# althonos/lightmotif

Hardware: AMD Instinct MI355X
Metric: scored positions/sec (higher is better)
Workload: dtype f32

## Files before the change

lightmotif_amd/build.py:

```python
from __future__ import annotations

import os
import shutil
import subprocess
import sys
from concurrent.futures import ThreadPoolExecutor
from pathlib import Path

PKG = Path(__file__).resolve().parent
CSRC = PKG / "csrc"
ROOT = PKG.parent
OBJ = CSRC / "_obj"
LIB = CSRC / "liblightmotif_hip.so"

ARCH = "gfx950"
FLAGS = [f"--offload-arch={ARCH}", "-O3", "-std=c++17", "-fPIC", "-ffp-contract=off",
         "-fno-slp-vectorize", "-fno-fast-math", "-Wall", "-Wno-unused-function",
         f"-I{ROOT / 'include'}", f"-I{CSRC}"]
INST = [(i, 4 * i + 1, 4 * i + 4) for i in range(9)]
LONG = list(range(40, 65, 4))
LONG_FLAGS = ["-mllvm", "-pragma-unroll-threshold=10000000"]
XLONG = list(range(72, 89, 8))
PAIR = [(65, 80), (81, 96), (97, 112), (113, 128)]
UNITS = ["score_plan.hip", "score_store.hip", "score_argmax.hip", "score_threshold.hip", "reduce.hip", "hits.hip", "seqset.hip", "seqset_best.hip", "fasta.hip", "dist.hip", "discrete.hip", "layout.hip", "scanmax.hip", "context.hip", "pssm.hip", "score_api.hip", "handles.hip",
         "hostptr.hip", "comm.hip"]
UNIT_FLAGS = {"seqset_best.hip": LONG_FLAGS}


def _hipcc() -> str:
    exe = shutil.which("hipcc") or "/opt/rocm/bin/hipcc"
    if not os.path.exists(exe):
        raise RuntimeError("hipcc not found: the HIP back-end cannot be built")
    return exe


def _newer(target: Path, deps: list[Path]) -> bool:
    if not target.exists():
        return True
    t = target.stat().st_mtime
    return any(d.stat().st_mtime > t for d in deps)


def _run(cmd: list[str]) -> None:
    r = subprocess.run(cmd, stdout=subprocess.PIPE, stderr=subprocess.STDOUT, text=True)
    if r.returncode != 0:
        raise RuntimeError("command failed: " + " ".join(cmd) + "\n" + r.stdout)
    if r.stdout.strip() and os.environ.get("LM_BUILD_VERBOSE"):
        print(r.stdout)


def build(force: bool = False, jobs: int | None = None) -> Path:
    hipcc = _hipcc()
    OBJ.mkdir(exist_ok=True)
    headers = list(CSRC.glob("*.hpp")) + [ROOT / "include" / "lightmotif_hip.h", Path(__file__)]
    cmds, objs = [], []
    for unit in UNITS:
        obj = OBJ / (unit + ".o")
        objs.append(obj)
        if force or _newer(obj, [CSRC / unit] + headers):
            cmds.append([hipcc, *FLAGS, *UNIT_FLAGS.get(unit, []), "-c", str(CSRC / unit), "-o", str(obj)])
    for inst, lo, hi in INST:
        obj = OBJ / f"score_inst_{inst}.o"
        objs.append(obj)
        if force or _newer(obj, [CSRC / "score_inst.hip"] + headers):
            cmds.append([hipcc, *FLAGS, f"-DLM_M_LO={lo}", f"-DLM_M_HI={hi}", f"-DLM_INST_ID={inst}",
                         "-c", str(CSRC / "score_inst.hip"), "-o", str(obj)])
    for m in LONG:
        obj = OBJ / f"score_long_inst_{m}.o"
        objs.append(obj)
        if force or _newer(obj, [CSRC / "score_long_inst.hip"] + headers):
            cmds.append([hipcc, *FLAGS, *LONG_FLAGS, f"-DLM_LONG_M={m}", "-c", str(CSRC / "score_long_inst.hip"),
                         "-o", str(obj)])
    for m in XLONG:
        obj = OBJ / f"score_xlong_inst_{m}.o"
        objs.append(obj)
        if force or _newer(obj, [CSRC / "score_xlong_inst.hip"] + headers):
            cmds.append([hipcc, *FLAGS, *LONG_FLAGS, f"-DLM_XLONG_M={m}", "-c", str(CSRC / "score_xlong_inst.hip"),
                         "-o", str(obj)])
    for lo, hi in PAIR:
        obj = OBJ / f"score_pair_inst_{lo}.o"
        objs.append(obj)
        if force or _newer(obj, [CSRC / "score_pair_inst.hip"] + headers):
            cmds.append([hipcc, *FLAGS, *LONG_FLAGS, f"-DLM_PAIR_LO={lo}", f"-DLM_PAIR_HI={hi}", "-c",
                         str(CSRC / "score_pair_inst.hip"), "-o", str(obj)])
    if cmds:
        def weight(cmd):
            text = " ".join(cmd)
            for m in LONG:
                if f"-DLM_LONG_M={m}" in text:
                    return 1000 + m
            for m in XLONG:
                if f"-DLM_XLONG_M={m}" in text:
                    return 900 + m
            for inst, lo, hi in INST:
                if f"-DLM_INST_ID={inst}" in text:
                    return 100 + hi
            if "score_pair_inst.hip" in text:
                return 90
            return 50 if "score_" in text else 0
        cmds.sort(key=weight, reverse=True)
        with ThreadPoolExecutor(max_workers=jobs or min(8, os.cpu_count() or 1)) as ex:
            list(ex.map(_run, cmds))
    if cmds or force or not LIB.exists():
        _run([hipcc, f"--offload-arch={ARCH}", "-shared", "-fPIC", "-o", str(LIB),
              *map(str, objs), "-ldl"])
        _audit(LIB)
    return LIB


# ... 15 lines not shown
```

lightmotif_amd/csrc/context.hip:

```cpp
#include <algorithm>
#include <sys/mman.h>
#include <cmath>
#include <cstdarg>
#include <cstdio>
#include <cstdlib>
#include <cctype>
#include <cstring>
#include <new>
#include <string>

#include "score_registry.hpp"

#include "lm_internal.hpp"

namespace lm {

static thread_local char g_err[512] = "";

int fail(int status, const char *fmt, ...)
{
    va_list ap;
    va_start(ap, fmt);
    vsnprintf(g_err, sizeof g_err, fmt, ap);
    va_end(ap);
// ... 213 lines not shown
    if (pinned_in_use) *pinned_in_use = used;
    if (budget) *budget = pool_budget();
    return LM_HIP_OK;
}

size_t lm_hip_stride(size_t cols, size_t elem_size)
{
    if (elem_size == 0)
        return 0;
    const size_t bytes = (cols * elem_size + 31) / 32 * 32;
    return bytes / elem_size;
}


namespace lm {
__global__ void clock_probe_kernel(unsigned long long window_ticks, unsigned long long *out)
{
    const unsigned long long r0 = __builtin_amdgcn_s_memrealtime();
    const unsigned long long c0 = __builtin_amdgcn_s_memtime();
    unsigned long long r1 = r0;
    while (r1 - r0 < window_ticks) {
        __builtin_amdgcn_s_sleep(127);
        r1 = __builtin_amdgcn_s_memrealtime();
    }
    const unsigned long long c1 = __builtin_amdgcn_s_memtime();
    if (threadIdx.x == 0) {
        out[0] = c1 - c0;
        out[1] = r1 - r0;
    }
}
}

int lm_hip_device_clock_mhz(int device, unsigned window_us, double *mhz)
{
    if (!mhz)
        return fail(LM_HIP_ERR_BAD_ARGS, "device_clock_mhz: null output");
    *mhz = 0.0;
    if (window_us == 0 || window_us > 2000000u)
        return fail(LM_HIP_ERR_BAD_ARGS, "device_clock_mhz: window of %u us (1 ... 2 000 000)", window_us);
    int n = 0;
    if (hipGetDeviceCount(&n) != hipSuccess || device < 0 || device >= n)
        return fail(LM_HIP_ERR_NO_DEVICE, "device %d out of range (%d devices)", device, n);
    DeviceGuard guard(device);
    int wall_khz = 0;
    LM_HIP_TRY(hipDeviceGetAttribute(&wall_khz, hipDeviceAttributeWallClockRate, device));
    if (wall_khz <= 0)
        return fail(LM_HIP_ERR_HIP, "device_clock_mhz: the device reports no constant-rate counter");
    struct Probe {
        hipStream_t stream = nullptr;
        unsigned long long *rec = nullptr;
    };
    static std::mutex probe_mu;
    static Probe probes[64];
    std::lock_guard<std::mutex> probe_lock(probe_mu);
    if (device >= 64)
        return fail(LM_HIP_ERR_BAD_ARGS, "device_clock_mhz: device ordinal %d", device);
    Probe &pr = probes[device];
    hipError_t e = hipSuccess;
    if (!pr.stream)
        e = hipStreamCreateWithFlags(&pr.stream, hipStreamNonBlocking);
    if (e == hipSuccess && !pr.rec)
        e = hipHostMalloc(reinterpret_cast<void **>(&pr.rec), 2 * sizeof(unsigned long long), hipHostMallocDefault);
    if (e == hipSuccess) {
        pr.rec[0] = pr.rec[1] = 0;
        hipLaunchKernelGGL(clock_probe_kernel, dim3(1), dim3(64), 0, pr.stream,
                           (unsigned long long)window_us * (unsigned long long)wall_khz / 1000ull, pr.rec);
        e = hipGetLastError();
    }
    if (e == hipSuccess)
        e = hipStreamSynchronize(pr.stream);
    const unsigned long long ticks = pr.rec ? pr.rec[0] : 0, ref = pr.rec ? pr.rec[1] : 0;
    if (e != hipSuccess)
        return fail(LM_HIP_ERR_HIP, "device_clock_mhz: %s", hipGetErrorString(e));
    if (ref == 0)
        return fail(LM_HIP_ERR_HIP, "device_clock_mhz: the constant-rate counter did not advance");
    *mhz = (double)ticks / (double)ref * (double)wall_khz / 1000.0;
    return LM_HIP_OK;
}


static const char *const kOptionNames[] = {"track_argmax", "xlong_store", "host_fold", "speculate_order", "suffix_argmax",
                                           "multi_motif", "quad_loads", "skip_unreachable", "pair_prefilter",
                                           "pair_prefilter_protein", "chunked_fused", "chunk_rows", "tiled",
                                           "suffix_occurrences", "prefilter", "sort_hits", "short_order", "time_scan", "drop_last", "block_prefilter", "list_scan_max", "poll_done"};

static int set_option(lm_hip_ctx *ctx, const char *name, double value)
{
    const bool on = value != 0;
    const std::string n(name);
    if (n == "track_argmax") ctx->track_argmax = on;
    else if (n == "xlong_store") ctx->xlong_store = on;
    else if (n == "host_fold") ctx->host_fold = on;
    else if (n == "speculate_order") ctx->speculate_order = on;
    else if (n == "sort_hits") ctx->sort_hits = on;
    else if (n == "time_scan") ctx->time_scan = on;
    else if (n == "poll_done") ctx->poll_done = on;
    else if (n == "list_scan_max") ctx->list_scan_max = on;
    else if (n == "drop_last") ctx->drop_last = on;
    else if (n == "short_order") ctx->short_order = on;
    else if (n == "suffix_argmax") ctx->suffix_argmax = on;
    else if (n == "multi_motif") ctx->multi_motif = on;
    else if (n == "quad_loads") ctx->quad_loads = on;
    else if (n == "skip_unreachable") ctx->skip_unreachable = on;
    else if (n == "pair_prefilter") ctx->pair_prefilter = on;
    else if (n == "block_prefilter") ctx->block_prefilter = on;
    else if (n == "pair_prefilter_protein") ctx->pair_prefilter_protein = on;
    else if (n == "chunked_fused") ctx->chunked_fused = on;
    else if (n == "tiled") ctx->tiled = on;
    else if (n == "prefilter") ctx->use_prefilter = on;
    else if (n == "xcd_remap") (void)on;
    else if (n == "chunk_rows") {
        if (!(value >= 64) || !(value <= 2147483648.0))
            return fail(LM_HIP_ERR_BAD_ARGS, "ctx_set_option: chunk_rows must be 64 ... 2^31");
        ctx->chunk_rows = (size_t)value;
    } else if (n == "suffix_occurrences") {
        ctx->suffix_occurrences = value > 0 ? value : 0;
    } else {
        return fail(LM_HIP_ERR_BAD_ARGS, "ctx_set_option: unknown option '%s'", name);
    }
    return LM_HIP_OK;
}

static void read_dev_switches(lm_hip_ctx *ctx)
{
#ifdef LM_HIP_DEV_SWITCHES
    for (const char *name : kOptionNames) {
        std::string env = "LM_HIP_";
        for (const char *c = name; *c; ++c)
            env += (char)toupper(*c);
        if (const char *e = getenv(env.c_str()))
            (void)set_option(ctx, name, atof(e));
    }
#else
    (void)ctx;
    (void)kOptionNames;
#endif
}

static int ctx_create(int device, void *stream, bool borrow, lm_hip_ctx **out)
{
    if (!out)
        return fail(LM_HIP_ERR_BAD_ARGS, "ctx_create: null output");
    *out = nullptr;
    if (const char *hole = score_registry_hole())
        return fail(LM_HIP_ERR_HIP, "%s", hole);
    int n = 0;
    if (hipGetDeviceCount(&n) != hipSuccess || n == 0)
        return fail(LM_HIP_ERR_NO_DEVICE, "no HIP device available");
    if (device < 0 || device >= n)
        return fail(LM_HIP_ERR_NO_DEVICE, "device %d out of range (%d devices)", device, n);
    hipDeviceProp_t prop;
    LM_HIP_TRY(hipGetDeviceProperties(&prop, device));
    if (strncmp(prop.gcnArchName, "gfx950", 6) != 0)
        return fail(LM_HIP_ERR_NO_DEVICE, "device %d is %s; this library is built for gfx950 only",
                    device, prop.gcnArchName);
    DeviceGuard guard(device);
    if (!guard.ok)
        return fail(LM_HIP_ERR_HIP, "hipSetDevice(%d) failed", device);
    lm_hip_ctx *ctx = new (std::nothrow) lm_hip_ctx();
    if (!ctx)
        return fail(LM_HIP_ERR_OOM, "out of host memory");
    ctx->device = device;
    ctx->num_cus = prop.multiProcessorCount;
    read_dev_switches(ctx);
    if (borrow) {
        ctx->stream = static_cast<hipStream_t>(stream);
        ctx->owns_stream = false;
    } else {
        hipError_t e = hipStreamCreateWithFlags(&ctx->stream, hipStreamNonBlocking);
        if (e != hipSuccess) {
            delete ctx;
            return fail(LM_HIP_ERR_HIP, "hipStreamCreate failed: %s", hipGetErrorString(e));
        }
        ctx->owns_stream = true;
    }
    hipError_t e = hipHostMalloc(&ctx->pinned, kPinnedBytes, hipHostMallocDefault);
    if (e != hipSuccess) {
        if (ctx->owns_stream)
            (void)hipStreamDestroy(ctx->stream);
        delete ctx;
        return fail(LM_HIP_ERR_OOM, "hipHostMalloc failed: %s", hipGetErrorString(e));
    }
    *out = ctx;
    return LM_HIP_OK;
// ... 151 lines not shown
```

lightmotif_amd/csrc/lm_internal.hpp:

```cpp
#pragma once

#include <hip/hip_runtime.h>

#include <cstddef>
#include <cstdint>
#include <mutex>
#include <string>
#include <vector>

#include "lightmotif_hip.h"

namespace lm {


int fail(int status, const char *fmt, ...) __attribute__((format(printf, 2, 3)));

#define LM_HIP_TRY(expr)                                                               \
    do {                                                                               \
        hipError_t _e = (expr);                                                        \
        if (_e != hipSuccess)                                                          \
            return ::lm::fail(_e == hipErrorOutOfMemory ? LM_HIP_ERR_OOM : LM_HIP_ERR_HIP, \
                              "%s failed: %s (%s:%d)", #expr, hipGetErrorString(_e),   \
                              __FILE__, __LINE__);                                     \
    } while (0)
// ... 19 lines not shown
    {
        if (prev >= 0)
            (void)hipSetDevice(prev);
    }
};


struct Scratch {
    void *ptr = nullptr;
    size_t bytes = 0;
    int reserve(size_t n);
    void release();
    void forget() { ptr = nullptr; bytes = 0; }
};

struct ArgmaxRecord {
    float value;
    int found;
    long long index;
};

constexpr size_t kPinnedBytes = 4u << 20;
struct PinnedRegion {
    size_t off, cap;
    constexpr size_t end() const { return off + cap; }
};
constexpr PinnedRegion kPinCounters{0, 16};
constexpr PinnedRegion kPinRecord{0, 64};
constexpr size_t kPinGenerationWordOff = sizeof(ArgmaxRecord);
constexpr PinnedRegion kPinArgmaxBatch{0, kPinnedBytes};
constexpr PinnedRegion kPinCandResults{16, kPinnedBytes / 2 - 16};
constexpr PinnedRegion kPinScanMaxState{0, 256};
constexpr PinnedRegion kPinListHead{256, kPinnedBytes / 2 - 256};
constexpr PinnedRegion kPinHitStaging{0, kPinnedBytes / 2};
constexpr PinnedRegion kPinHitReadback{0, 256u << 10};
constexpr PinnedRegion kPinFoldRecords{4096, kPinnedBytes - 4096};
constexpr PinnedRegion kPinU8Out{4096, kPinnedBytes / 2 - 4096};
constexpr PinnedRegion kPinUploadHead{kPinnedBytes / 2, kPinnedBytes / 2};
constexpr PinnedRegion kPinCommBlock{0, kPinnedBytes};
constexpr PinnedRegion kPinCommGather{0, kPinnedBytes / 2};

static_assert(kPinRecord.end() <= kPinFoldRecords.off, "single-job argmax: the record and its generation word lie before the wavefront records");
static_assert(kPinCounters.end() <= kPinCandResults.off, "candidate-route argmax: the counters lie before the results");
static_assert(kPinCandResults.end() <= kPinUploadHead.off, "candidate-route argmax: the results end where the uploaded head begins");
static_assert(kPinCounters.end() <= kPinListHead.off, "Scanner::max by list: the counters lie before the head of the list");
static_assert(kPinHitStaging.end() <= kPinUploadHead.off, "fused threshold: the kernels' staging ends where the uploaded head begins");
static_assert(kPinHitReadback.end() <= kPinHitStaging.end(), "the exact ordering's read-back stays inside the staging of the speculative one");
static_assert(kPinListHead.end() <= kPinUploadHead.off && kPinU8Out.end() <= kPinUploadHead.off, "the lower half's users stay in the lower half");

void *result_alloc(size_t bytes);
void result_free(void *p);

}


struct lm_hip_ctx {
    int device = 0;
    hipStream_t stream = nullptr;
    bool owns_stream = false;
    hipStream_t aux_stream = nullptr;
    hipEvent_t fork_event = nullptr, join_event = nullptr;
    hipStream_t copy_stream = nullptr;
    hipEvent_t tile_copied[2] = {nullptr, nullptr}, tile_consumed[2] = {nullptr, nullptr};
    std::mutex mu;
    lm::Scratch scratch;
    lm::Scratch scratch2;
    lm::Scratch scan_buf;
    lm::Scratch chunk_scores;
    size_t chunk_rows = 1u << 22;
    bool chunked_fused = true;
    void *pinned = nullptr;
    unsigned fold_generation = 0;
    unsigned *d_ticket = nullptr;
    unsigned *d_short = nullptr;
    unsigned short_generation = 0;
    bool poll_done = false;
    bool short_dirty = false;
    size_t rows_per_stream = 0;
    bool use_prefilter = true;
    bool pair_prefilter = true;
    bool block_prefilter = true;
    bool pair_prefilter_protein = false;
    bool quad_loads = true;
    bool track_argmax = true;
    bool xlong_store = true;
    bool host_fold = true;
    bool speculate_order = true;
    bool sort_hits = true;
    bool time_scan = false;
    hipEvent_t scan_ev[4] = {nullptr, nullptr, nullptr, nullptr};
    bool scan_timed = false;
    int scan_marks = 0;
    float last_scan_kernel_ms = -1.0f;
    float last_phase_ms[4] = {-1.0f, -1.0f, -1.0f, -1.0f};
    unsigned last_scan_rows = 0, last_scan_lds_bytes = 0;
    bool list_scan_max = true;
    bool drop_last = true;
    bool short_order = true;
    bool suffix_argmax = true;
    bool multi_motif = true;
    bool skip_unreachable = true;
    bool tiled = true;
    double suffix_occurrences = 0;
    int num_cus = 256;
    unsigned long long last_hit_count = 0;
    unsigned long long last_cand_count = 0;
    const char *last_kernel = "";
    lm::Scratch u8_tables;
    std::vector<uint8_t> u8_key;
};

namespace lm {
template <class T>
inline T *pinned_at(const lm_hip_ctx *ctx, PinnedRegion r, size_t count = 1, size_t byte_off = 0)
{
    if (byte_off + count * sizeof(T) > r.cap)
        return nullptr;
    return reinterpret_cast<T *>(static_cast<char *>(ctx->pinned) + r.off + byte_off);
}

template <class T>
inline int read_back(lm_hip_ctx *ctx, hipStream_t st, const void *d_src, T *out)
{
    static_assert(sizeof(T) <= kPinCounters.cap, "read_back is for a counter");
    T *h = pinned_at<T>(ctx, kPinCounters);
    LM_HIP_TRY(hipMemcpyAsync(h, d_src, sizeof(T), hipMemcpyDeviceToHost, st));
    LM_HIP_TRY(hipStreamSynchronize(st));
    *out = *h;
    return LM_HIP_OK;
}
inline int read_back_counters(lm_hip_ctx *ctx, hipStream_t st, const void *d_counters, unsigned long long out[2])
{
    struct Pair { unsigned long long hits, candidates; } p{};
    LM_TRY(read_back(ctx, st, d_counters, &p));
    out[0] = p.hits;
    out[1] = p.candidates;
    return LM_HIP_OK;
}

inline unsigned next_generation(unsigned &g) { return ++g ? g : ++g; }
inline bool poll_generation(const volatile unsigned *word, unsigned generation, unsigned spins = 1u << 20)
{
    for (unsigned spin = 0; spin < spins; ++spin) {
        if (__atomic_load_n(word, __ATOMIC_ACQUIRE) == generation)
            return true;
#if defined(__x86_64__) && !defined(__HIP_DEVICE_COMPILE__)
        __builtin_ia32_pause();
#endif
    }
    return false;
}
struct FoldSlots {
    uint4 *records;
    unsigned generation;
};
inline FoldSlots begin_fold(lm_hip_ctx *ctx, size_t nrec, bool want_records = true)
{
    FoldSlots f{want_records ? pinned_at<uint4>(ctx, kPinFoldRecords, nrec + 1) : nullptr, next_generation(ctx->fold_generation)};
    if (f.records)
        for (size_t r = 0; r <= nrec; ++r)
            reinterpret_cast<volatile unsigned long long *>(f.records)[2 * r] = 0ull;
    return f;
}

inline int scan_timer_begin(lm_hip_ctx *ctx, hipStream_t st)
{
// ... 270 lines not shown
```

lightmotif_amd/csrc/score_kernels.hpp:

```cpp
#pragma once
#include <type_traits>

#include <hip/hip_runtime.h>

#include <cstddef>
#include <cstdint>

#include "lm_internal.hpp"

namespace lm {

constexpr int kBlock = 256;
constexpr int kStreamsPerBlock = kBlock / 32;
constexpr int kMaxFastM = 36;
constexpr int kMaxLongM = 64;
constexpr int kMaxStoreM = 88;
constexpr int kMaxPairM = 128;

constexpr bool lds_wide(int k) { return k > 16; }
constexpr int table_stride(int m, int wide = 0) { return wide ? 4 * ((m + 3) / 4) + 2 : 4 * (((m + 3) / 4) | 1); }
typedef float lm_f32x2_t __attribute__((ext_vector_type(2)));
typedef const volatile __attribute__((address_space(3))) lm_f32x2_t *lm_lds_b64_ptr;
typedef unsigned lm_u32x2_t __attribute__((ext_vector_type(2)));
typedef const volatile __attribute__((address_space(3))) lm_u32x2_t *lm_lds_u64_ptr;
typedef unsigned lm_u32x4_t __attribute__((ext_vector_type(4)));
typedef const __attribute__((address_space(3))) lm_u32x4_t *lm_lds_u128_ptr;
typedef const __attribute__((address_space(3))) unsigned *lm_lds_u32_ptr;
__device__ __forceinline__ void lds_zero_based(const void *dynamic_lds)
{
    if ((unsigned)(size_t)(const __attribute__((address_space(3))) char *)dynamic_lds != 0u)
        __builtin_trap();
}

enum : int { MODE_STORE = 0, MODE_ARGMAX = 1, MODE_THRESHOLD = 2, MODE_STORE_ARGMAX = 3, MODE_CONTINUE = 4,
             MODE_STORE_TRACK = 5 };
enum : int { SLOT_STORE = MODE_STORE, SLOT_ARGMAX = MODE_ARGMAX, SLOT_THRESHOLD = MODE_THRESHOLD, SLOT_STORE_QL,
             SLOT_STORE_ARGMAX, SLOT_CONTINUE, SLOT_STORE_C16, SLOT_STORE_TRACK, kRegistrySlots };
constexpr bool mode_stores(int mode)
{
    return mode == MODE_STORE || mode == MODE_STORE_ARGMAX || mode == MODE_CONTINUE || mode == MODE_STORE_TRACK;
}
constexpr bool mode_tracks_best(int mode)
{
    return mode == MODE_ARGMAX || mode == MODE_STORE_ARGMAX || mode == MODE_STORE_TRACK;
}
constexpr bool mode_tracks_cell(int mode) { return mode == MODE_ARGMAX || mode == MODE_STORE_TRACK; }

struct __attribute__((aligned(16))) HitRecord {
    unsigned long long key;
    float value;
    unsigned pad;
};

struct __attribute__((aligned(16))) Candidate {
    unsigned long long key;
    unsigned nrows;
    unsigned col;
};

struct BatchParams {
    const void *table;
    ArgmaxRecord *block_best;
    float threshold;
    unsigned td;
    unsigned long long job_key;
};

struct FusedOut {
    ArgmaxRecord *block_best;
    float threshold;
    unsigned long long *hit_count;
    HitRecord *hits;
    unsigned long long job_key;
    unsigned long long hit_capacity;
    unsigned long long key_rows;
    unsigned long long *cand_count;
    Candidate *cands;
    unsigned long long cand_capacity;
    const BatchParams *batch;
    unsigned lead_rows;
    unsigned *ticket;
    ArgmaxRecord *final_out;
    ArgmaxRecord *final_host;
    int first_cell_rule;
    unsigned generation;
    uint4 *host_records;
};

__device__ __forceinline__ void best_merge(float &v, long long &i, float ov, long long oi)
{
    if (oi >= 0 && (i < 0 || ov > v || (ov == v && oi > i))) {
        v = ov;
        i = oi;
    }
}

__device__ __forceinline__ void best_wave_reduce(float &v, long long &i)
{
#pragma unroll
    for (int off = 32; off > 0; off >>= 1) {
        const float ov = __shfl_xor(v, off);
        const long long oi = __shfl_xor(i, off);
        best_merge(v, i, ov, oi);
    }
}

__device__ __forceinline__ float wave_max_dpp(float v)
{
    auto step = [](float x, auto ctrl) {
        const int moved = __builtin_amdgcn_update_dpp(__builtin_bit_cast(int, x), __builtin_bit_cast(int, x),
                                                      decltype(ctrl)::value, 0xf, 0xf, false);
        return __builtin_fmaxf(x, __builtin_bit_cast(float, moved));
    };
    v = step(v, std::integral_constant<int, 0xb1>{});
    v = step(v, std::integral_constant<int, 0x4e>{});
    v = step(v, std::integral_constant<int, 0x141>{});
    v = step(v, std::integral_constant<int, 0x140>{});
    const float r0 = __builtin_bit_cast(float, __builtin_amdgcn_readlane(__builtin_bit_cast(int, v), 0));
    const float r1 = __builtin_bit_cast(float, __builtin_amdgcn_readlane(__builtin_bit_cast(int, v), 16));
    const float r2 = __builtin_bit_cast(float, __builtin_amdgcn_readlane(__builtin_bit_cast(int, v), 32));
// ... 750 lines not shown
```

lightmotif_amd/csrc/score_plan.hip:

```cpp
#include <cstdio>
#include <cstring>
#include <mutex>

#include "score_launch.hpp"

namespace lm {


static ScoreC32Launcher g_c32[kMaxStoreM + 1][kRegistrySlots];
static ScoreC32Launcher g_c32w[kMaxStoreM + 1][kRegistrySlots];
static PrefilterLauncher g_prew[kMaxFastM + 1];
static PrefilterLauncher g_preblk[kMaxFastM + 1];
static ScoreU8Launcher g_u8w[kMaxFastM + 1];
static PrefilterLauncher g_pre[kMaxFastM + 1];
static PrefilterLauncher g_pre2[kMaxPairM + 1];
static PrefilterLauncher g_pre2_protein[kMaxFastM + 1];
static ScoreU8Launcher g_u8[kMaxFastM + 1];
static ScoreU8Launcher g_u8_pairs[kMaxFastM + 1];
static PrefilterMultiLauncher g_pre2_multi[kMaxFastM + 1];
static char g_c32_names[kMaxStoreM + 1][3][32];
static char g_hole[96];
static std::once_flag g_c32_once;

static void find_hole()
{
    auto check = [](bool filled, const char *row, int m) {
        if (!filled && !g_hole[0])
            snprintf(g_hole, sizeof g_hole, "kernel registry: no %s kernel for M = %d (a unit of the build is not registered)", row, m);
    };
    for (int m = 1; m <= kMaxStoreM; ++m)
        if (m <= kMaxFastM || (m <= kMaxLongM ? m % 4 == 0 : m % 8 == 0))
            check(g_c32[m][SLOT_STORE] && g_c32w[m][SLOT_STORE], "store", m);
    for (int m = 2; m <= kMaxPairM; ++m)
        check(g_pre2[m], "pair scan", m);
    for (int m = 1; m <= kMaxFastM; ++m)
        check(g_pre[m] && g_prew[m] && g_u8[m] && g_u8w[m], "one-symbol scan or u8", m);
}

static void init_registry()
{
    const KernelRegistry r{g_c32, g_pre, g_pre2, g_pre2_protein, g_u8, g_u8_pairs, g_pre2_multi, g_c32w, g_prew, g_u8w, g_preblk};
#define LM_CALL_UNIT(f) f(r);
    LM_REGISTERING_UNITS(LM_CALL_UNIT)
#undef LM_CALL_UNIT
    find_hole();
    for (int m = 0; m <= kMaxStoreM; ++m)
        for (int mode = 0; mode < 3; ++mode)
            snprintf(g_c32_names[m][mode], sizeof g_c32_names[m][mode], "score_c32<%d,%d>", m, mode);
}

const char *score_registry_hole()
{
    std::call_once(g_c32_once, init_registry);
    return g_hole[0] ? g_hole : nullptr;
}

ScoreC32Launcher score_c32_lookup(int M, int slot, bool wide)
{
    std::call_once(g_c32_once, init_registry);
    if (M < 1 || M > kMaxStoreM || slot < 0 || slot >= kRegistrySlots)
        return nullptr;
    if (slot == SLOT_STORE_C16 && M > kMaxFastM)
        return nullptr;
    return (wide ? g_c32w : g_c32)[M][slot];
}

PrefilterLauncher score_c32_prefilter_lookup(int M, bool wide, bool blocks)
{
    std::call_once(g_c32_once, init_registry);
    return (M >= 1 && M <= kMaxFastM) ? (wide ? (blocks ? g_preblk[M] : g_prew[M]) : g_pre[M]) : nullptr;
}

PrefilterLauncher score_c32_prefilter2_lookup(int M, int K)
{
    std::call_once(g_c32_once, init_registry);
    if (M < 1 || M > (K == 5 ? kMaxPairM : kMaxFastM))
        return nullptr;
    return K == 5 ? g_pre2[M] : K == 21 ? g_pre2_protein[M] : nullptr;
}

PrefilterMultiLauncher score_c32_prefilter2_multi_lookup(int M)
{
    std::call_once(g_c32_once, init_registry);
    return (M >= 1 && M <= kMaxFastM) ? g_pre2_multi[M] : nullptr;
}

ScoreU8Launcher score_c32_lookup_u8(int M, bool pairs, bool wide)
{
    std::call_once(g_c32_once, init_registry);
    if (M < 1 || M > kMaxFastM)
        return nullptr;
    return pairs ? g_u8_pairs[M] : wide ? g_u8w[M] : g_u8[M];
}

const char *score_c32_name(int M, int mode)
{
    std::call_once(g_c32_once, init_registry);
    return (M >= 0 && M <= kMaxStoreM && mode >= 0 && mode < 3) ? g_c32_names[M][mode] : "score_c32";
}


ExactMotif exact_motif(const lm_hip_pssm *p, const uint8_t *d_seq)
{
    if (p->m <= (size_t)kMaxFastM)
        return ExactMotif{p->m, p->d_table, 0u};
    if (p->parts.size() == 1 && p->parts[0].m <= (size_t)kMaxLongM && reinterpret_cast<uintptr_t>(d_seq) % 4 == 0)
        return ExactMotif{p->parts[0].m, p->parts[0].d_table, (unsigned)p->parts[0].lead};
    return ExactMotif{};
}

C32Plan plan_c32(const lm_hip_ctx *ctx, const ScoreArgs &a, bool store, int prefilter, size_t batch)
{
    const size_t m = prefilter == 0 ? exact_motif(a.pssm, a.d_seq).m : a.pssm->m;
    const MotifShape ms{m, a.pssm->k, a.pssm->d_image2 != nullptr};
    return plan_c32(ctx, ms, a, store, prefilter, batch);
}

C32Plan plan_c32(const lm_hip_ctx *ctx, const MotifShape &ms, const ScoreArgs &a, bool store,
                        int prefilter, size_t batch, unsigned long long default_rows, bool allow16)
{
    C32Plan p;
    const size_t K = ms.k;
    const size_t M = prefilter == 2   ? (size_t)prefilter2_ring((int)ms.m)
                     : prefilter == 1 ? (size_t)prefilter_mp((int)ms.m, lds_wide((int)K))
                                      : ms.m;
    const size_t extra = prefilter == 2 ? 2 : 1;
    const unsigned long long n = a.row_end - a.row_begin;
    const bool c16 = allow16 && store && prefilter == 0 && a.cols == 16;
    if ((a.cols != 32 && !c16) || a.seq_stride != 32 || (store && a.out_stride != a.cols))
        return p;
    if (ms.m < 1 || ms.m > (size_t)(prefilter == 0 ? (store ? kMaxStoreM : kMaxLongM) : (prefilter == 2 && K == 5) ? kMaxPairM : kMaxFastM) || n < M + extra)
        return p;
    if (prefilter == 0 && ms.m > (size_t)kMaxFastM && (ms.m % 4 != 0 || reinterpret_cast<uintptr_t>(a.d_seq) % 4 != 0))
        return p;
    if (prefilter == 2 && ((K != 5 && !(K == 21 && ctx->pair_prefilter_protein)) || !ms.pair_table || ms.m < 2 ||
                           reinterpret_cast<uintptr_t>(a.d_seq) % 4 != 0))
        return p;
    const size_t lds = prefilter == 2   ? (size_t)prefilter2_image_dw((int)ms.m, (int)K) * 4
                       : prefilter == 1 ? (size_t)prefilter_image_dw((int)ms.m, (int)K) * 4
                                        : std::max<size_t>(K * table_stride((int)M, lds_wide((int)K)) * sizeof(float), 64);
    if (lds > 60 * 1024)
        return p;
    unsigned long long target = ctx->rows_per_stream ? ctx->rows_per_stream
                                : default_rows         ? default_rows
                                : !store               ? 1024
                                : prefilter != 0       ? 64
                                : ms.m > 26            ? 6 * M
                                                       : std::max<size_t>(3 * M, 24);
    const unsigned long long want_streams =
        std::max<unsigned long long>((unsigned long long)ctx->num_cus * (store ? 64 : 128) / batch, 64);
    if (n / target < want_streams)
        target = std::max<unsigned long long>(n / want_streams, 1);
    target = std::min<unsigned long long>(target, 1ull << 30);
    unsigned long long q = std::max<unsigned long long>((target + M / 2) / M, 1);
    if (q * M + extra > n)
        q = (n - extra) / M;
    if (q < 1)
        return p;
    p.T = q * M + extra;
    p.nstreams = (n + p.T - 1) / p.T;
    const unsigned long long per_block = c16 ? 2 * kStreamsPerBlock : kStreamsPerBlock;
    p.grid = dim3((unsigned)((p.nstreams + per_block - 1) / per_block));
    p.lds = lds;
    p.ok = true;
    return p;
}

dim3 generic_grid(const lm_hip_ctx *ctx, unsigned long long ncells)
{
    unsigned long long blocks = (ncells + kBlock - 1) / kBlock;
    const unsigned long long cap = (unsigned long long)ctx->num_cus * 32;
    return dim3((unsigned)std::max<unsigned long long>(std::min(blocks, cap), 1));
}

size_t generic_lds(const lm_hip_pssm *p, int *use_lds)
// ... 205 lines not shown
```

lightmotif_amd/csrc/score_registry.hpp:

```cpp
#pragma once

#include "score_u8.hpp"

namespace lm {

struct KernelRegistry {
    ScoreC32Launcher (*c32)[kRegistrySlots];
    PrefilterLauncher *pre, *pre2;
    PrefilterLauncher *pre2_protein;
    ScoreU8Launcher *u8, *u8_pairs;
    PrefilterMultiLauncher *pre2_multi;
    ScoreC32Launcher (*c32w)[kRegistrySlots];
    PrefilterLauncher *prew;
    ScoreU8Launcher *u8w;
    PrefilterLauncher *preblk;
};

#define LM_REGISTERING_UNITS(X)                                                                                        \
    X(register_score_c32_0) X(register_score_c32_1) X(register_score_c32_2) X(register_score_c32_3)                    \
    X(register_score_c32_4) X(register_score_c32_5) X(register_score_c32_6) X(register_score_c32_7)                    \
    X(register_score_c32_8)                                                                                            \
    X(register_score_c32_long_40) X(register_score_c32_long_44) X(register_score_c32_long_48)                          \
    X(register_score_c32_long_52) X(register_score_c32_long_56) X(register_score_c32_long_60)                          \
    X(register_score_c32_long_64)                                                                                      \
    X(register_score_c32_xlong_72) X(register_score_c32_xlong_80) X(register_score_c32_xlong_88)                       \
    X(register_score_pair_65) X(register_score_pair_81) X(register_score_pair_97) X(register_score_pair_113)
#define LM_DECLARE_UNIT(f) void f(const KernelRegistry &r);
LM_REGISTERING_UNITS(LM_DECLARE_UNIT)
#undef LM_DECLARE_UNIT

#define LM_CAT2(a, b) a##b
#define LM_CAT(a, b) LM_CAT2(a, b)

const char *score_registry_hole();

ScoreC32Launcher score_c32_lookup(int M, int slot, bool wide = false);
const char *score_c32_name(int M, int mode);
PrefilterLauncher score_c32_prefilter_lookup(int M, bool wide = false, bool blocks = false);
PrefilterLauncher score_c32_prefilter2_lookup(int M, int K = 5);
PrefilterMultiLauncher score_c32_prefilter2_multi_lookup(int M);
ScoreU8Launcher score_c32_lookup_u8(int M, bool pairs, bool wide);

}
```

lightmotif_amd/csrc/score_store.hip:

```cpp
#include <algorithm>
#include <cstring>

#include "score_launch.hpp"

namespace lm {


static unsigned long long store_rows_hint(size_t m_kernel, size_t cols)
{
    return (cols == 32 && m_kernel == 12) ? 12 : 0;
}

static unsigned tiled_plan(const lm_hip_ctx *ctx, const ScoreArgs &a, unsigned long long *tr_out, size_t *lds_out)
{
    if (!ctx->tiled)
        return 0;
    const size_t tab_bytes = (a.pssm->m * a.pssm->k * 4 + 15) / 16 * 16;
    const size_t budget = 40 * 1024;
    const unsigned long long n = a.row_end - a.row_begin;
    if (!(a.pssm->m >= 1 && tab_bytes + (a.pssm->m + 8) * a.cols <= budget && a.cols <= 4096))
        return 0;
    unsigned long long tr = (budget - tab_bytes) / a.cols - (a.pssm->m - 1);
    tr = std::min<unsigned long long>(tr / kTiledStrip * kTiledStrip, 2048);
    while (tr > kTiledStrip * 4 && (n + tr - 1) / tr < (unsigned long long)ctx->num_cus * 4)
        tr = (tr / 2 + kTiledStrip - 1) / kTiledStrip * kTiledStrip;
    if (tr < (unsigned long long)kTiledStrip)
        return 0;
    *tr_out = tr;
    *lds_out = tab_bytes + (tr + a.pssm->m - 1) * a.cols + 16;
    return (unsigned)((n + tr - 1) / tr);
}

unsigned tiled_records(const lm_hip_ctx *ctx, const ScoreArgs &a)
{
    unsigned long long tr = 0;
    size_t lds = 0;
    return tiled_plan(ctx, a, &tr, &lds);
}

int launch_score_store(lm_hip_ctx *ctx, const ScoreArgs &a)
{
    FusedOut fo{};
    const bool wide = lds_wide((int)a.pssm->k);
    const bool dwords = ctx->quad_loads && reinterpret_cast<uintptr_t>(a.d_seq) % 4 == 0;
    if (dwords && a.pssm->d_table_pad) {
        const size_t mp = a.pssm->m + a.pssm->lead;
        const MotifShape ms{mp, a.pssm->k, false};
        const C32Plan pp = plan_c32(ctx, ms, a, true, 0, 1, store_rows_hint(mp, a.cols), true);
        ScoreC32Launcher pfn = a.cols == 16 ? score_c32_lookup((int)mp, SLOT_STORE_C16, wide) : score_c32_lookup((int)mp, SLOT_STORE_QL, wide);
        if (pp.ok && pfn) {
            fo.lead_rows = (unsigned)a.pssm->lead;
            ctx->last_kernel = score_c32_name((int)mp, MODE_STORE);
            LM_HIP_TRY(pfn(pp.grid, pp.lds, ctx->stream, a.d_seq, a.pssm->d_table_pad,
                                                    (int)a.pssm->k, a.row_begin, a.row_end, pp.T, pp.nstreams, a.d_out,
                                                    fo));
            return LM_HIP_OK;
        }
    }
    const bool c16 = a.cols == 16 && dwords && score_c32_lookup((int)a.pssm->m, SLOT_STORE_C16, wide);
    const C32Plan p = a.pssm->m <= (size_t)kMaxFastM ? plan_c32(ctx, MotifShape{a.pssm->m, a.pssm->k, false}, a, true, 0, 1,
                                                                  store_rows_hint(a.pssm->m, a.cols), c16)
                                                      : C32Plan{};
    if (p.ok) {
        ScoreC32Launcher fn = score_c32_lookup((int)a.pssm->m, SLOT_STORE, wide);
        if (dwords && score_c32_lookup((int)a.pssm->m, SLOT_STORE_QL, wide))
            fn = score_c32_lookup((int)a.pssm->m, SLOT_STORE_QL, wide);
        if (c16)
            fn = score_c32_lookup((int)a.pssm->m, SLOT_STORE_C16, wide);
        ctx->last_kernel = score_c32_name((int)a.pssm->m, MODE_STORE);
        LM_HIP_TRY(fn(p.grid, p.lds, ctx->stream, a.d_seq, a.pssm->d_table, (int)a.pssm->k,
                      a.row_begin, a.row_end, p.T, p.nstreams, a.d_out, fo));
        return LM_HIP_OK;
    }
    if (!a.pssm->parts.empty() && a.cols == 32 && a.seq_stride == 32 && a.out_stride == 32 &&
        reinterpret_cast<uintptr_t>(a.d_seq) % 4 == 0 && a.row_end - a.row_begin > a.pssm->parts[0].m) {
        const unsigned long long n = a.row_end - a.row_begin;
        bool ok = true;
        for (size_t i = 0; i < a.pssm->parts.size() && ok; ++i) {
            const lm_hip_pssm::Part &part = a.pssm->parts[i];
            const MotifShape ms{part.m, a.pssm->k, false};
            ScoreArgs sa = a;
            sa.d_seq = a.d_seq + part.off * a.seq_stride;
            const C32Plan p = plan_c32(ctx, ms, sa, true);
            if (!p.ok) {
                ok = false;
                break;
            }
            FusedOut pfo = fo;
            pfo.lead_rows = (unsigned)part.lead;
            if (i == 0) {
                ScoreC32Launcher fn = score_c32_lookup((int)part.m, SLOT_STORE_QL, wide);
                if (!fn)
                    fn = score_c32_lookup((int)part.m, SLOT_STORE, wide);
                LM_HIP_TRY(fn(p.grid, p.lds, ctx->stream, sa.d_seq, part.d_table, (int)a.pssm->k, a.row_begin, a.row_end,
                              p.T, p.nstreams, a.d_out, pfo));
                continue;
            }
            const unsigned long long nfull = n / p.T;
            if (nfull) {
                const dim3 grid((unsigned)((nfull + kStreamsPerBlock - 1) / kStreamsPerBlock));
                LM_HIP_TRY(score_c32_lookup((int)part.m, SLOT_CONTINUE, wide)(grid, p.lds, ctx->stream, sa.d_seq, part.d_table,
                                                                  (int)a.pssm->k, a.row_begin, a.row_begin + nfull * p.T,
                                                                  p.T, nfull, a.d_out, pfo));
            }
            if (nfull * p.T < n) {
                const unsigned long long r0 = a.row_begin + nfull * p.T;
                const unsigned long long cells = (a.row_end - r0) * a.cols;
                hipLaunchKernelGGL(score_continue_cells<0>, dim3((unsigned)((cells + kBlock - 1) / kBlock)), dim3(kBlock), 0,
                                   ctx->stream, sa.d_seq, (unsigned long long)a.seq_stride, (int)a.cols,
                                   a.pssm->d_dense + part.off * a.pssm->k, (int)(part.m - part.lead), (int)a.pssm->k, r0,
                                   (unsigned long long)a.row_end, a.d_out + (r0 - a.row_begin) * a.out_stride,
                                   (unsigned long long)a.out_stride);
                LM_HIP_TRY(hipGetLastError());
            }
        }
        if (ok) {
            ctx->last_kernel = a.pssm->parts.size() == 1 ? score_c32_name((int)a.pssm->parts[0].m, MODE_STORE)
                                                         : "score_c32_sliced";
            return LM_HIP_OK;
        }
    }
    unsigned long long tr = 0;
    size_t lds = 0;
    const unsigned grid_x = tiled_plan(ctx, a, &tr, &lds);
    if (grid_x) {
        ctx->last_kernel = "score_tiled";
        const dim3 grid(grid_x);
// ... 436 lines not shown
```

Baseline: 1032.

## Add quad-hopping store kernel using DPP lane shifts for short motifs

Adds a new store-mode kernel for motif lengths that are multiples of four (up to the short-family limit). Each lane carries a running partial-sum array, and DPP cross-lane moves shift partial sums between neighbouring lanes, so every lane adds one weight per motif row per step. Symbol bytes are fetched through raw buffer loads with alignbit, and results are written with nontemporal 128-bit stores. With default settings the kernel is only chosen for M=16 on 32-column, 16-byte-aligned layouts. It aims to cut redundant per-position table reads, at the cost of a large unrolled kernel with higher register pressure and a fragile indexing scheme.

```diff
diff --git a/lightmotif_amd/build.py b/lightmotif_amd/build.py
--- a/lightmotif_amd/build.py
+++ b/lightmotif_amd/build.py
@@ -22,9 +22,9 @@
 LONG_FLAGS = ["-mllvm", "-pragma-unroll-threshold=10000000"]
 XLONG = list(range(72, 89, 8))
 PAIR = [(65, 80), (81, 96), (97, 112), (113, 128)]
-UNITS = ["score_plan.hip", "score_store.hip", "score_argmax.hip", "score_threshold.hip", "reduce.hip", "hits.hip", "seqset.hip", "seqset_best.hip", "fasta.hip", "dist.hip", "discrete.hip", "layout.hip", "scanmax.hip", "context.hip", "pssm.hip", "score_api.hip", "handles.hip",
+UNITS = ["score_hop_inst.hip", "score_plan.hip", "score_store.hip", "score_argmax.hip", "score_threshold.hip", "reduce.hip", "hits.hip", "seqset.hip", "seqset_best.hip", "fasta.hip", "dist.hip", "discrete.hip", "layout.hip", "scanmax.hip", "context.hip", "pssm.hip", "score_api.hip", "handles.hip",
          "hostptr.hip", "comm.hip"]
-UNIT_FLAGS = {"seqset_best.hip": LONG_FLAGS}
+UNIT_FLAGS = {"seqset_best.hip": LONG_FLAGS, "score_hop_inst.hip": LONG_FLAGS}
 
 
 def _hipcc() -> str:
diff --git a/lightmotif_amd/csrc/context.hip b/lightmotif_amd/csrc/context.hip
--- a/lightmotif_amd/csrc/context.hip
+++ b/lightmotif_amd/csrc/context.hip
@@ -319,7 +319,7 @@
 static const char *const kOptionNames[] = {"track_argmax", "xlong_store", "host_fold", "speculate_order", "suffix_argmax",
                                            "multi_motif", "quad_loads", "skip_unreachable", "pair_prefilter",
                                            "pair_prefilter_protein", "chunked_fused", "chunk_rows", "tiled",
-                                           "suffix_occurrences", "prefilter", "sort_hits", "short_order", "time_scan", "drop_last", "block_prefilter", "list_scan_max", "poll_done"};
+                                           "suffix_occurrences", "prefilter", "sort_hits", "short_order", "time_scan", "drop_last", "block_prefilter", "list_scan_max", "poll_done", "store_hop"};
 
 static int set_option(lm_hip_ctx *ctx, const char *name, double value)
 {
@@ -337,6 +337,7 @@
     else if (n == "short_order") ctx->short_order = on;
     else if (n == "suffix_argmax") ctx->suffix_argmax = on;
     else if (n == "multi_motif") ctx->multi_motif = on;
+    else if (n == "store_hop") ctx->store_hop = value == 2 ? 2 : on ? 1 : 0;
     else if (n == "quad_loads") ctx->quad_loads = on;
     else if (n == "skip_unreachable") ctx->skip_unreachable = on;
     else if (n == "pair_prefilter") ctx->pair_prefilter = on;
diff --git a/lightmotif_amd/csrc/lm_internal.hpp b/lightmotif_amd/csrc/lm_internal.hpp
--- a/lightmotif_amd/csrc/lm_internal.hpp
+++ b/lightmotif_amd/csrc/lm_internal.hpp
@@ -125,6 +125,7 @@
     bool block_prefilter = true;
     bool pair_prefilter_protein = false;
     bool quad_loads = true;
+    int store_hop = 1;
     bool track_argmax = true;
     bool xlong_store = true;
     bool host_fold = true;
diff --git a/lightmotif_amd/csrc/score_hop.hpp b/lightmotif_amd/csrc/score_hop.hpp
--- /dev/null
+++ b/lightmotif_amd/csrc/score_hop.hpp
@@ -0,0 +1,235 @@
+#pragma once
+#include <utility>
+
+#include "score_kernels.hpp"
+
+namespace lm {
+
+constexpr int hop_drain_steps(int m) { return 8 * (m / 8); }
+constexpr int hop_min_rows(int m) { return hop_drain_steps(m) > 8 ? hop_drain_steps(m) : 8; }
+
+constexpr int hop_min_waves(int m) { return m <= 20 ? 6 : 4; }
+
+typedef float lm_f32x4_t __attribute__((ext_vector_type(4)));
+typedef const __attribute__((address_space(3))) lm_f32x4_t *lm_lds_f128_ptr;
+
+__device__ __forceinline__ float hop_add(const float below, const float w)
+{
+    const int moved = __builtin_amdgcn_update_dpp(0, __builtin_bit_cast(int, below), 0x93 , 0xf, 0xf, true);
+    return __builtin_bit_cast(float, moved) + w;
+}
+
+template <int M, int C0, int C1, int BYTE, int EI>
+__device__ __forceinline__ void hop_step(float (&A)[M], float (&E)[8], const unsigned syms, const unsigned tsb)
+{
+    const unsigned row = byte_times<BYTE>(syms, tsb);
+    float w[M];
+#pragma unroll
+    for (int c = C0; c < C1; ++c) {
+        const lm_f32x4_t v = *(lm_lds_f128_ptr)(size_t)(row + 16u * c);
+        w[4 * c + 0] = v.x;
+        w[4 * c + 1] = v.y;
+        w[4 * c + 2] = v.z;
+        w[4 * c + 3] = v.w;
+    }
+#pragma unroll
+    for (int j = 4 * C1 - 1; j >= 4 * C0; --j) {
+        if (j == 0) {
+            A[0] = 0.0f + w[0];
+        } else {
+            const float r = hop_add(A[j - 1], w[j]);
+            if (j == M - 1)
+                E[EI] = r;
+            else
+                A[j] = r;
+        }
+    }
+    __builtin_amdgcn_sched_barrier(0);
+}
+
+struct HopLoads {
+    __amdgpu_buffer_rsrc_t rsrc;
+    unsigned next;
+    __device__ __forceinline__ unsigned load()
+    {
+        const unsigned d = (unsigned)__builtin_amdgcn_raw_buffer_load_b32(rsrc, (int)next, 0, 0);
+        next += 128;
+        return d;
+    }
+};
+
+template <int RS, bool LOAD>
+__device__ __forceinline__ void hop_block(unsigned (&D)[4], unsigned &syms, const unsigned sh, HopLoads &ld)
+{
+    syms = __builtin_amdgcn_alignbit(D[RS], D[(RS + 3) % 4], sh);
+    if (LOAD)
+        D[(RS + 3) % 4] = ld.load();
+}
+
+template <int U6>
+__device__ __forceinline__ void hop_store(const float (&E)[8], float *&op, const bool odd, const bool high)
+{
+    const float e0 = E[U6 & 7], e1 = E[(U6 + 1) & 7], e2 = E[(U6 + 2) & 7], e3 = E[(U6 + 3) & 7], e4 = E[(U6 + 4) & 7],
+                e5 = E[(U6 + 5) & 7], e6 = E[(U6 + 6) & 7];
+    const float x[6] = {odd ? e1 : e0, odd ? e2 : e1, odd ? e3 : e2, odd ? e4 : e3, odd ? e5 : e4, odd ? e6 : e5};
+    lm_f32x4_t v;
+    v.x = high ? x[2] : x[0];
+    v.y = high ? x[3] : x[1];
+    v.z = high ? x[4] : x[2];
+    v.w = high ? x[5] : x[3];
+    __builtin_nontemporal_store(v, reinterpret_cast<lm_f32x4_t *>(op));
+    op += 4 * 32;
+}
+
+struct HopState {
+    unsigned D[4];
+    unsigned syms;
+    unsigned sh, tsb;
+    bool odd, high;
+    HopLoads ld;
+    float *op;
+};
+
+template <int M, int TAU>
+__device__ __forceinline__ void hop_fill_step(float (&A)[M], float (&E)[8], HopState &s)
+{
+    if constexpr (TAU % 4 == 0)
+        hop_block<(TAU / 4) % 4, true>(s.D, s.syms, s.sh, s.ld);
+    constexpr int c1 = (TAU - 1) / 4 + 1 < M / 4 ? (TAU - 1) / 4 + 1 : M / 4;
+    hop_step<M, 0, c1, TAU % 4, ((TAU - M) % 8 + 8) % 8>(A, E, s.syms, s.tsb);
+}
+template <int M, int... TAU1>
+__device__ __forceinline__ void hop_fill(float (&A)[M], float (&E)[8], HopState &s, std::integer_sequence<int, TAU1...>)
+{
+    (hop_fill_step<M, TAU1 + 1>(A, E, s), ...);
+}
+
+template <int M, int S>
+__device__ __forceinline__ void hop_main_step(float (&A)[M], float (&E)[8], HopState &s)
+{
+    constexpr int u = 3 + S;
+    if constexpr (u % 4 == 0)
+        hop_block<((u + M) / 4) % 4, true>(s.D, s.syms, s.sh, s.ld);
+    hop_step<M, 0, M / 4, u % 4, u % 8>(A, E, s.syms, s.tsb);
+    if constexpr (u % 4 == 2)
+        hop_store<(u - 6 + 8) % 8>(E, s.op, s.odd, s.high);
+}
+template <int M, int... S>
+__device__ __forceinline__ void hop_main(float (&A)[M], float (&E)[8], HopState &s, std::integer_sequence<int, S...>)
+{
+    (hop_main_step<M, S>(A, E, s), ...);
+}
+
+template <int M, int I>
+__device__ __forceinline__ void hop_drain_step(float (&A)[M], float (&E)[8], HopState &s)
+{
+    constexpr int v = I + 3 - hop_drain_steps(M);
+    constexpr int vp = v + 64;
+    if constexpr (vp % 4 == 0)
+        hop_block<((I + 3 + M) / 4) % 4, (v + 12 <= -2)>(s.D, s.syms, s.sh, s.ld);
+    constexpr int need = v + M - 3;
+    constexpr int c0 = need <= 0 ? 0 : need / 4;
+    hop_step<M, c0, M / 4, vp % 4, vp % 8>(A, E, s.syms, s.tsb);
+    if constexpr (vp % 4 == 2)
+        hop_store<(vp - 6) % 8>(E, s.op, s.odd, s.high);
+}
+template <int M, int... I>
+__device__ __forceinline__ void hop_drain(float (&A)[M], float (&E)[8], HopState &s, std::integer_sequence<int, I...>)
+{
+    (hop_drain_step<M, I>(A, E, s), ...);
+}
+
+template <int M>
+__global__ __attribute__((amdgpu_flat_work_group_size(1, kBlock), amdgpu_waves_per_eu(hop_min_waves(M)))) void score_c32_hop(
+    const uint8_t *__restrict__ seq, const float *__restrict__ table, const int K, const unsigned long long row_begin,
+    const unsigned long long row_end, const unsigned long long T, const unsigned long long nstreams, float *__restrict__ out,
+    const FusedOut fo)
+{
+    static_assert(M % 4 == 0 && M >= 4 && M <= kMaxFastM, "whole 4-row symbol blocks, the short family");
+    extern __shared__ __attribute__((aligned(16))) char lds_raw[];
+    lds_zero_based(lds_raw);
+    {
+        float4 *dst = reinterpret_cast<float4 *>(lds_raw);
+        const float4 *src = reinterpret_cast<const float4 *>(table);
+        const int n4 = K * table_stride(M) / 4;
+        for (int i = threadIdx.x; i < n4; i += kBlock)
+            dst[i] = src[i];
+    }
+    __syncthreads();
+
+    const int lane = threadIdx.x & 63;
+    const int col = lane & 31, q = col & 3;
+    unsigned long long stream = ((unsigned long long)blockIdx.x * (kBlock / 64) + (threadIdx.x >> 6)) * 2 + (lane >> 5);
+    if (stream >= nstreams)
+        stream = nstreams - 1;
+    unsigned long long o0 = row_begin + stream * T;
+    if (o0 + T > row_end)
+        o0 = row_end - T;
+    const long long lead = (long long)fo.lead_rows;
+    const long long in0 = (long long)o0 - lead;
+
+    HopState s;
+    {
+        const unsigned lo = __builtin_amdgcn_readfirstlane((unsigned)(unsigned long long)in0);
+        const unsigned hi = __builtin_amdgcn_readfirstlane((unsigned)((unsigned long long)in0 >> 32));
+        long long base_row = (long long)(((unsigned long long)hi << 32) | lo);
+        if (base_row < 0)
+            base_row = 0;
+        const unsigned long long end_row = row_end + (unsigned long long)(M - lead) - 1;
+        const unsigned long long bytes = (end_row - (unsigned long long)base_row) * 32;
+        s.ld.rsrc = __builtin_amdgcn_make_buffer_rsrc(const_cast<uint8_t *>(seq) + base_row * 32, 0,
+                                                      (int)(bytes < 0xffffffffull ? bytes : 0xffffffffull), 0x00020000);
+        s.ld.next = (unsigned)((in0 + q - base_row) * 32) + (unsigned)(col >> 2) * 4u;
+    }
+    s.sh = 24u - 8u * (unsigned)q;
+    s.tsb = table_stride(M) * 4u;
+    const unsigned phi = (unsigned)(q + 1) & 3u;
+    s.odd = (phi & 1u) != 0;
+    s.high = (phi & 2u) != 0;
+    s.op = out + ((o0 - row_begin) + phi) * 32 + (col >> 2) * 4;
+
+    float A[M], E[8];
+#pragma unroll
+    for (int j = 0; j < M; ++j)
+        A[j] = 0.0f;
+#pragma unroll
+    for (int j = 0; j < 8; ++j)
+        E[j] = 0.0f;
+    if (in0 + q >= 0) {
+        s.D[0] = s.ld.load();
+    } else {
+        s.D[0] = 0;
+        s.ld.next += 128;
+    }
+    s.D[1] = s.ld.load();
+    s.D[2] = s.ld.load();
+    s.D[3] = 0;
+    hop_block<0, true>(s.D, s.syms, s.sh, s.ld);
+
+    hop_fill<M>(A, E, s, std::make_integer_sequence<int, M + 2>{});
+    const unsigned halves = (unsigned)((T - hop_drain_steps(M)) / 8);
+    for (unsigned it = 0; it < halves / 2; ++it)
+        hop_main<M>(A, E, s, std::make_integer_sequence<int, 16>{});
+    if (halves & 1u) {
+        hop_main<M>(A, E, s, std::make_integer_sequence<int, 8>{});
+        unsigned t = s.D[0];
+        s.D[0] = s.D[2];
+        s.D[2] = t;
+        t = s.D[1];
+        s.D[1] = s.D[3];
+        s.D[3] = t;
+    }
+    hop_drain<M>(A, E, s, std::make_integer_sequence<int, hop_drain_steps(M)>{});
+}
+
+template <int M>
+hipError_t score_c32_hop_launch(dim3 grid, size_t lds_bytes, hipStream_t stream, const uint8_t *seq, const float *table, int K,
+                                unsigned long long row_begin, unsigned long long row_end, unsigned long long T,
+                                unsigned long long nstreams, float *out, FusedOut fo)
+{
+    hipLaunchKernelGGL((score_c32_hop<M>), grid, dim3(kBlock), lds_bytes, stream, seq, table, K, row_begin, row_end, T, nstreams,
+                       out, fo);
+    return hipGetLastError();
+}
+
+}
diff --git a/lightmotif_amd/csrc/score_hop_inst.hip b/lightmotif_amd/csrc/score_hop_inst.hip
--- /dev/null
+++ b/lightmotif_amd/csrc/score_hop_inst.hip
@@ -0,0 +1,16 @@
+#include "score_hop.hpp"
+#include "score_registry.hpp"
+
+namespace lm {
+
+template <int M>
+static void register_hop(const KernelRegistry &r)
+{
+    r.c32[M][SLOT_STORE_HOP] = &score_c32_hop_launch<M>;
+    if constexpr (M + 4 <= kMaxFastM)
+        register_hop<M + 4>(r);
+}
+
+void register_score_hop(const KernelRegistry &r) { register_hop<4>(r); }
+
+}
diff --git a/lightmotif_amd/csrc/score_kernels.hpp b/lightmotif_amd/csrc/score_kernels.hpp
--- a/lightmotif_amd/csrc/score_kernels.hpp
+++ b/lightmotif_amd/csrc/score_kernels.hpp
@@ -35,7 +35,7 @@
 enum : int { MODE_STORE = 0, MODE_ARGMAX = 1, MODE_THRESHOLD = 2, MODE_STORE_ARGMAX = 3, MODE_CONTINUE = 4,
              MODE_STORE_TRACK = 5 };
 enum : int { SLOT_STORE = MODE_STORE, SLOT_ARGMAX = MODE_ARGMAX, SLOT_THRESHOLD = MODE_THRESHOLD, SLOT_STORE_QL,
-             SLOT_STORE_ARGMAX, SLOT_CONTINUE, SLOT_STORE_C16, SLOT_STORE_TRACK, kRegistrySlots };
+             SLOT_STORE_ARGMAX, SLOT_CONTINUE, SLOT_STORE_C16, SLOT_STORE_TRACK, SLOT_STORE_HOP, kRegistrySlots };
 constexpr bool mode_stores(int mode)
 {
     return mode == MODE_STORE || mode == MODE_STORE_ARGMAX || mode == MODE_CONTINUE || mode == MODE_STORE_TRACK;
diff --git a/lightmotif_amd/csrc/score_plan.hip b/lightmotif_amd/csrc/score_plan.hip
--- a/lightmotif_amd/csrc/score_plan.hip
+++ b/lightmotif_amd/csrc/score_plan.hip
@@ -2,6 +2,7 @@
 #include <cstring>
 #include <mutex>
 
+#include "score_hop.hpp"
 #include "score_launch.hpp"
 
 namespace lm {
@@ -31,6 +32,8 @@
     for (int m = 1; m <= kMaxStoreM; ++m)
         if (m <= kMaxFastM || (m <= kMaxLongM ? m % 4 == 0 : m % 8 == 0))
             check(g_c32[m][SLOT_STORE] && g_c32w[m][SLOT_STORE], "store", m);
+    for (int m = 4; m <= kMaxFastM; m += 4)
+        check(g_c32[m][SLOT_STORE_HOP], "quad-hopping store", m);
     for (int m = 2; m <= kMaxPairM; ++m)
         check(g_pre2[m], "pair scan", m);
     for (int m = 1; m <= kMaxFastM; ++m)
@@ -91,6 +94,26 @@
     if (M < 1 || M > kMaxFastM)
         return nullptr;
     return pairs ? g_u8_pairs[M] : wide ? g_u8w[M] : g_u8[M];
+}
+
+static unsigned long long store_hop_table(int M)
+{
+    switch (M) {
+    case 16: return 64;
+    default: return 0;
+    }
+}
+
+unsigned long long store_hop_rows(int M, int mode, unsigned long long forced)
+{
+    if (mode == 0 || M < 4 || M > kMaxFastM || M % 4 != 0 || !score_c32_lookup(M, SLOT_STORE_HOP))
+        return 0;
+    unsigned long long rows = store_hop_table(M);
+    if (!rows && mode < 2)
+        return 0;
+    rows = forced ? forced : rows ? rows : 64;
+    rows = std::max<unsigned long long>((rows + 4) / 8 * 8, (unsigned long long)hop_min_rows(M));
+    return std::min<unsigned long long>(rows, 1ull << 20);
 }
 
 const char *score_c32_name(int M, int mode)
diff --git a/lightmotif_amd/csrc/score_registry.hpp b/lightmotif_amd/csrc/score_registry.hpp
--- a/lightmotif_amd/csrc/score_registry.hpp
+++ b/lightmotif_amd/csrc/score_registry.hpp
@@ -24,7 +24,8 @@
     X(register_score_c32_long_52) X(register_score_c32_long_56) X(register_score_c32_long_60)                          \
     X(register_score_c32_long_64)                                                                                      \
     X(register_score_c32_xlong_72) X(register_score_c32_xlong_80) X(register_score_c32_xlong_88)                       \
-    X(register_score_pair_65) X(register_score_pair_81) X(register_score_pair_97) X(register_score_pair_113)
+    X(register_score_pair_65) X(register_score_pair_81) X(register_score_pair_97) X(register_score_pair_113)                   \
+    X(register_score_hop)
 #define LM_DECLARE_UNIT(f) void f(const KernelRegistry &r);
 LM_REGISTERING_UNITS(LM_DECLARE_UNIT)
 #undef LM_DECLARE_UNIT
@@ -40,5 +41,6 @@
 PrefilterLauncher score_c32_prefilter2_lookup(int M, int K = 5);
 PrefilterMultiLauncher score_c32_prefilter2_multi_lookup(int M);
 ScoreU8Launcher score_c32_lookup_u8(int M, bool pairs, bool wide);
+unsigned long long store_hop_rows(int M, int mode, unsigned long long forced);
 
 }
diff --git a/lightmotif_amd/csrc/score_store.hip b/lightmotif_amd/csrc/score_store.hip
--- a/lightmotif_amd/csrc/score_store.hip
+++ b/lightmotif_amd/csrc/score_store.hip
@@ -43,6 +43,23 @@
     FusedOut fo{};
     const bool wide = lds_wide((int)a.pssm->k);
     const bool dwords = ctx->quad_loads && reinterpret_cast<uintptr_t>(a.d_seq) % 4 == 0;
+    if (ctx->store_hop && dwords && !wide && a.cols == 32 && a.seq_stride == 32 && a.out_stride == 32 &&
+        reinterpret_cast<uintptr_t>(a.d_out) % 16 == 0) {
+        const bool pad = a.pssm->d_table_pad != nullptr;
+        const size_t mp = a.pssm->m + (pad ? a.pssm->lead : 0);
+        const unsigned long long T = mp <= (size_t)kMaxFastM ? store_hop_rows((int)mp, ctx->store_hop, ctx->rows_per_stream) : 0;
+        const unsigned long long n = a.row_end - a.row_begin;
+        if (T && n >= T) {
+            const unsigned long long nstreams = (n + T - 1) / T;
+            const dim3 grid((unsigned)((nstreams + kStreamsPerBlock - 1) / kStreamsPerBlock));
+            const size_t lds = std::max<size_t>(a.pssm->k * table_stride((int)mp) * sizeof(float), 64);
+            fo.lead_rows = pad ? (unsigned)a.pssm->lead : 0u;
+            ctx->last_kernel = score_c32_name((int)mp, MODE_STORE);
+            LM_HIP_TRY(score_c32_lookup((int)mp, SLOT_STORE_HOP)(grid, lds, ctx->stream, a.d_seq, pad ? a.pssm->d_table_pad : a.pssm->d_table,
+                                                                (int)a.pssm->k, a.row_begin, a.row_end, T, nstreams, a.d_out, fo));
+            return LM_HIP_OK;
+        }
+    }
     if (dwords && a.pssm->d_table_pad) {
         const size_t mp = a.pssm->m + a.pssm->lead;
         const MotifShape ms{mp, a.pssm->k, false};
```

New measurement: 1032, median of 2. Within noise of the previous version (-0.0%).
